# huggingface/gym-genesis

Measured on AMD Instinct MI355X. Metric: env-steps/sec (num_envs x sim-steps/sec), CubePick-v0 @ num_envs=4096, higher is better.
Workload: dtype f32

## Files before the change

gym-genesis_amd/csrc/mir_api.hip:

```cpp
#include <hip/hip_runtime.h>
#include <hip/hip_ext.h>

#include <cstdio>
#include <cstdlib>
#include <cstring>
#include <ctime>
#include <new>

#include "mir_host.h"
#include "mir_model.h"
#include "mir_scene.h"
#include "mir_spec_pick.h"
#include "mir_step.h"
#include "mir_step64.h"

using namespace mir_host;

static_assert((int)RK_FULL == (int)STEP_FULL && (int)RK_POST == (int)STEP_POST && (int)RK_ROTATED == (int)STEP_ROTATED && (int)RK_HEAVY48 == (int)STEP_HEAVY48 &&
              (int)RK_POST48 == (int)STEP_POST48 && (int)RK_ROTATED_LIST == (int)STEP_ROTATED_LIST, "mir_route.h numbers its launches like StepKind");

namespace {

thread_local char g_err[512] = "";

// ... 122 lines not shown
  snprintf(g_err, sizeof g_err, fmt, detail);
  return code;
}
int mir_host::hip_fail(hipError_t e, const char* what) {
  snprintf(g_err, sizeof g_err, "%s: %s", what, hipGetErrorString(e));
  return MIR_E_HIP;
}

int mir_host::launch(MirScene* h, const Outs& o, void* stream) {
  int rc;
  const bool sense = o.mode == 1 && (o.cf_ncon || o.cf_flags || o.cf_ids || o.cf_geom || o.cf_force || o.cf_link);
  if (!step_keeps_pre(o.kind) && o.mode != 2 && !sense) h->pre_valid = 0;
  const bool integrates = o.mode == 0 && step_integrates(o.kind);
  if (integrates && !step_completes_counted_step(o.kind)) h->state_version++;
  const bool wr_poses = o.poses || (h->poses_live && integrates);
  if (o.mode == 2 && o.poses) h->poses_current = 1;
  else if (integrates && o.kind != STEP_LIST48) h->poses_current = (h->kernel == 64 || wr_poses) && !o.ar.episode_len;
  if (h->kernel == 16) {
    StepArgs a;
    memset(&a, 0, sizeof a);
    a.model = h->dm;
    a.qpos = h->qpos; a.qvel = h->qvel; a.target = h->target; a.qacc_ws = h->qacc_ws;
    a.poses = wr_poses ? h->poses : nullptr;
    a.early_stats = h->early_stats; a.no_early_mask = h->no_early_mask;
    a.term_bad = h->pin_dev ? reinterpret_cast<uint32_t*>(h->pin_dev + h->pin_flag_off + 16) : nullptr;
    a.term_wstride = h->term_wstride;
    a.diag = (o.diag && h->diag_on) ? h->diag : nullptr;
    a.B = h->B; a.qst = h->hm.qstride; a.nu = h->hm.nu; a.features = (h->hm.has_convex ? FEAT_CONVEX : 0) | (h->hm.use_sap ? FEAT_CONVEX | FEAT_SAP : 0) | ((h->spec_pick && (!wr_poses || step_spec_stores_poses(o.kind))) ? FEAT_SPEC : 0);
    a.action = o.action; a.agent_pos = o.agent_pos; a.env_state = o.env_state; a.reward = o.reward; a.terminated = o.terminated;
    a.out_M = o.out_M; a.out_bias = o.out_bias; a.out_qas = o.out_qas; a.out_qacc = o.out_qacc; a.out_xpos = o.out_xpos; a.out_xquat = o.out_xquat;
    a.rows = o.rows; a.row_stride = o.row_stride; a.mode = o.mode; a.n_steps = o.n_steps; a.prof = o.prof;
    a.act_step = o.act_step; a.rows_step = o.rows_step; a.ar = o.ar;
    a.term_host = o.term_host; a.term_tag = o.term_tag; a.done_ticket = o.done_ticket; a.done_flag = o.done_flag; a.done_seq = o.done_seq;
    a.kind = o.kind; a.pre = h->pre;
    a.exact = o.exact; a.over_cap = o.over_cap;
    a.pre_big = step_uses_pre_big(o.kind) ? h->xc.res.pre_big : nullptr;
    a.next_host = o.next_host;
    a.cf_ncon = o.cf_ncon; a.cf_flags = o.cf_flags; a.cf_ids = o.cf_ids; a.cf_geom = o.cf_geom; a.cf_force = o.cf_force; a.cf_link = o.cf_link;
    if (step_forward_only(o.kind)) a.features &= ~FEAT_SPEC;
    if (o.env_list) { a.env_list = o.env_list; a.B = o.nlist; }
    if (o.kind == STEP_LIST48) a.term_wstride = 1;
    rc = mir_launch_step(&a, (hipStream_t)stream);
  } else {
    StepArgs64 a;
    memset(&a, 0, sizeof a);
    a.model = h->dm64;
    a.qpos = h->qpos; a.qvel = h->qvel; a.target = h->target; a.qacc_ws = h->qacc_ws;
// ... 54 lines not shown
namespace {

int create_device_state(MirScene* h, const GeomTab& gt, const float* row, size_t row_bytes) {
  DeviceGuard guard(h->device);
  const PlumbTab& t = h->pt;
  const size_t B = (size_t)h->B;
  const size_t qst = t.qst, vst = t.vst, pst = t.pst;
  HIPCHK(hipMalloc((void**)&h->dm, sizeof(DevModel)));
  HIPCHK(hipMalloc((void**)&h->dm64, sizeof(DevModel64)));
  HIPCHK(hipMalloc((void**)&h->dpt, sizeof(PlumbTab)));
  HIPCHK(hipMalloc((void**)&h->dgeom, sizeof(GeomTab)));
  HIPCHK(hipMalloc((void**)&h->qpos, B * qst * sizeof(float)));
  HIPCHK(hipMalloc((void**)&h->qvel, B * vst * sizeof(float)));
  HIPCHK(hipMalloc((void**)&h->target, B * vst * sizeof(float)));
  HIPCHK(hipMalloc((void**)&h->qacc_ws, B * vst * sizeof(float)));
  HIPCHK(hipMalloc((void**)&h->diag, B * 4 * sizeof(int32_t)));
  HIPCHK(hipMalloc((void**)&h->poses, B * 2 * pst * 4 * sizeof(float)));
  HIPCHK(hipMalloc((void**)&h->fkvalid, B * sizeof(int32_t)));
  HIPCHK(hipMalloc((void**)&h->done_ticket, 64));
  HIPCHK(hipMalloc((void**)&h->scratch_row, row_bytes));
  if (h->kernel == 16) HIPCHK(hipMalloc((void**)&h->pre, B * K16_PRE_STRIDE * sizeof(float)));
  h->spec_pick = h->kernel == 16 && SpecPick::matches(h->hm) && !getenv("MIR_NO_SPEC");
  h->no_early_mask = getenv("MIR_NO_EARLY_MASK") ? 1 : 0;
  HIPCHK(hipMalloc((void**)&h->early_stats, early_words(h) * sizeof(uint32_t)));
  HIPCHK(hipMemset(h->early_stats, 0, early_words(h) * sizeof(uint32_t)));
  if (h->kernel == 64) {
    h->cost_stride = (int)(((B + 63) / 64) * 64);
    HIPCHK(hipMalloc((void**)&h->cost, 2 * (size_t)h->cost_stride));
    HIPCHK(hipMemset(h->cost, 0, 2 * (size_t)h->cost_stride));
  }
  h->term_wstride = h->kernel == 16 ? 16 : 0;
  h->pin_flag_off = h->term_wstride ? ((B + 3) / 4) * 4 * (size_t)h->term_wstride : ((B + 63) / 64) * 64;
  h->pin_flag_off = (h->pin_flag_off + 63) / 64 * 64;
  const size_t pin_bytes = h->pin_flag_off + 64;
  HIPCHK(hipHostMalloc((void**)&h->pin_host, pin_bytes, hipHostMallocMapped | hipHostMallocCoherent));
  memset(h->pin_host, 0, pin_bytes);
  HIPCHK(hipHostGetDevicePointer((void**)&h->pin_dev, h->pin_host, 0));
  HIPCHK(hipMemcpy(h->dm, &h->hm, sizeof(DevModel), hipMemcpyHostToDevice));
  HIPCHK(hipMemcpy(h->dm64, &h->hm64, sizeof(DevModel64), hipMemcpyHostToDevice));
  HIPCHK(hipMemcpy(h->dpt, &h->pt, sizeof(PlumbTab), hipMemcpyHostToDevice));
  HIPCHK(hipMemcpy(h->dgeom, &gt, sizeof(GeomTab), hipMemcpyHostToDevice));
  for (int g = 0; g < gt.ngeom; g++) h->render_round |= gt.g_type[g] == MIR_GEOM_SPHERE || gt.g_type[g] == MIR_GEOM_CAPSULE;
  HIPCHK(hipMemcpy(h->scratch_row, row, row_bytes, hipMemcpyHostToDevice));
  hipLaunchKernelGGL(k_fill_rows, dim3(nblk((long)B * qst)), dim3(TPB), 0, 0, h->qpos, h->scratch_row, (int)qst, h->B);
  HIPCHK(hipGetLastError());
  HIPCHK(hipMemset(h->qvel, 0, B * vst * sizeof(float)));
// ... 829 lines not shown
```

gym-genesis_amd/csrc/mir_scene.h:

```cpp
#pragma once
#include <stdint.h>

#include "mir_model.h"
#include "mir_model64.h"
#include "mir_route.h"

struct ExactRes {
  int32_t *ovf_list_host, *ovf_list_dev;
  uint8_t *ovf_term_host, *ovf_term_dev;
  int32_t *perm_host[2], *perm_dev[2];
  void* ovf_stream;
  void* ovf_event;
  int ovf_event_live;
  void* ovf_waited_stream;
  void* main_event;
  void* light_event;
  float* pre_big;
  uint32_t *next_host, *next_dev;
  unsigned long long* xr_stats;
  int32_t* xr_count;
  int32_t *xr_list, *xr_list2, *xr_start;
  unsigned long long xr_calls;
};

// ... 6 lines not shown
  ExactStats stats;
};

struct MirScene {
  int device;
  int B;
  int kernel;
  DevModel hm;
  DevModel64 hm64;
  HostConsts hc;
  PlumbTab pt;
  int nbody, nv, nq, nu, ngeom, npair, agent_dim, env_dim;
  DevModel* dm;
  DevModel64* dm64;
  PlumbTab* dpt;
  GeomTab* dgeom;
  float *qpos, *qvel, *target, *qacc_ws, *poses;
  int32_t *diag, *fkvalid;
  uint8_t* cost = nullptr;
  int cost_par = 0;
  int cost_stride = 0;
  uint32_t* early_stats = nullptr;
  int no_early_mask = 0;
  int spec_pick = 0;
  float* prims;
  int* bins = nullptr;
  size_t bins_cap = 0;
  int render_th = 0;
  int render_generic = 0;
  int render_round = 0;
  unsigned long long* zbuf = nullptr;
  size_t zbuf_cap = 0;
  unsigned* vis = nullptr;
  size_t vis_cap = 0;
  unsigned long long state_version = 0;
  int poses_live = 0;
  int poses_current = 0;
  float* scratch_row;
  uint8_t* pin_host;
  size_t pin_flag_off = 0;
  int term_wstride = 0;
  uint8_t* pin_dev;
  uint32_t* done_ticket;
  uint32_t seq;
  uint32_t tag;
  int sync_mode;
// ... 22 lines not shown
```

gym-genesis_amd/csrc/mir_step.h:

```cpp
#pragma once
#include <hip/hip_runtime.h>
#include <stdint.h>

#include "mir_model.h"

enum : int { FEAT_PLAIN = 0 , FEAT_CONVEX = 1, FEAT_SAP = 2, FEAT_SPEC = 4 };

enum StepKind : int {
  STEP_SINGLE = 0,
  STEP_LOOP = 1,
  STEP_FULL = 2,
  STEP_PRE = 3,
  STEP_POST = 4,
  STEP_ROTATED = 5,
  STEP_LIST48 = 6,
  STEP_HEAVY48 = 7,
  STEP_POST48 = 9,
  STEP_PRE48 = 10,
  STEP_ROTATED_LIST = 11,
  STEP_XR16 = 12,
  STEP_XR48 = 13,
  STEP_SENSE48 = 14,
};

constexpr int step_cpl(int k) { return (k == STEP_LIST48 || k == STEP_HEAVY48 || k == STEP_POST48 || k == STEP_PRE48 || k == STEP_XR48 || k == STEP_SENSE48) ? 3 : 1; }
constexpr bool step_big(int k) { return step_cpl(k) > 1; }
constexpr bool step_fused_next_pre(int k) { return k == STEP_LIST48; }
constexpr bool step_packed(int k) { return step_big(k) || k == STEP_ROTATED_LIST; }
constexpr bool step_rotated(int k) { return k == STEP_ROTATED || k == STEP_POST48 || k == STEP_ROTATED_LIST; }
constexpr bool step_first_pass_only(int k) { return k == STEP_POST48 || k == STEP_ROTATED_LIST; }
constexpr bool step_pre_only(int k) { return k == STEP_PRE || k == STEP_PRE48; }
constexpr bool step_post_only(int k) { return k == STEP_POST; }
constexpr bool step_forward_only(int k) { return k == STEP_SENSE48; }
constexpr bool step_has_loop(int k) { return k == STEP_LOOP || k == STEP_FULL || k == STEP_XR16; }
constexpr bool step_rows_only(int k) { return k == STEP_LOOP || k == STEP_XR16; }
constexpr bool step_exact_rollout(int k) { return k == STEP_XR16 || k == STEP_XR48; }
constexpr int step_waves(int k) { return (step_has_loop(k) || step_post_only(k)) ? 1 : 2; }
constexpr int step_block(int k) { return 64 * step_waves(k); }
constexpr int step_wpe_min(int k) { return (step_rotated(k) && !step_big(k)) ? 2 : 1; }
constexpr int step_wpe_max(int k) { return (step_rotated(k) && !step_big(k)) ? 2 : (step_big(k) ? 1 : 10); }
constexpr bool step_defers(int k) { return k == STEP_SINGLE || k == STEP_POST || k == STEP_ROTATED || k == STEP_ROTATED_LIST || k == STEP_XR16 || step_big(k); }
constexpr bool step_reads_env_list(int k) { return k == STEP_PRE || k == STEP_ROTATED_LIST || step_big(k); }
constexpr bool step_sends_host_bytes(int k) { return k != STEP_LOOP && !step_forward_only(k); }
constexpr bool step_early_bytes_in_solver(int k) { return k == STEP_SINGLE || k == STEP_ROTATED || k == STEP_POST48 || k == STEP_ROTATED_LIST; }
constexpr bool step_spec_stores_poses(int k) { return step_rotated(k) || step_big(k); }
constexpr bool step_integrates(int k) { return !step_pre_only(k) && !step_forward_only(k); }
constexpr bool step_keeps_pre(int k) { return step_pre_only(k) || k == STEP_LIST48; }
constexpr bool step_completes_counted_step(int k) { return k == STEP_LIST48 || k == STEP_ROTATED_LIST; }
constexpr bool step_uses_pre_big(int k) { return k == STEP_LIST48 || k == STEP_POST48 || k == STEP_PRE48; }

struct StepArgs {
  const DevModel* model;
  float* qpos;
  float* qvel;
  float* target;
  float* qacc_ws;
  float* poses;
  const float* action;
  float* agent_pos;
  float* env_state;
  float* reward;
  uint8_t* terminated;
  uint8_t* term_host;
// ... 17 lines not shown
  int B;
  int qst, nu;
  int mode;
  int n_steps;
  int features;
  int kind;
  float* pre;
  uint32_t* early_stats;
  uint32_t* term_bad;
  int no_early_mask;
  int term_wstride;
  int exact;
  int over_cap;
  const int32_t* env_list;
  float* pre_big;
  uint32_t* next_host;
  int32_t* xr_list;
  int32_t* xr_count;
  int32_t* xr_list2;
  int32_t* xr_count2;
  int32_t* xr_start;
  unsigned long long* xr_stats;
  int xr_step;
  int32_t* cf_ncon;
  uint8_t* cf_flags;
  int32_t* cf_ids;
  float* cf_geom;
  float* cf_force;
  float* cf_link;
};
#ifndef XR_TIER2
#define XR_TIER2 (1 << 20)
#endif
#define K48_HEAD 0
#define K48_CMETA 4
#define K48_JB (K48_CMETA + 4 * MIR_MAX_CONTACT)
#define K48_STRIDE (((K48_JB + 48 * MIR_MAX_CONTACT) + 15) / 16 * 16)
#define K48_MAGIC 0x42494721
#define K16_PRE_MROW 0
#define K16_PRE_BIAS 256
#define K16_PRE_HEAD 272
#define K16_PRE_CMETA 276
#define K16_PRE_JB (K16_PRE_CMETA + 4 * K16_MAX_CONTACT)
#define K16_PRE_STRIDE (((K16_PRE_JB + 52 * K16_MAX_CONTACT) + 15) / 16 * 16)


// ... 3 lines not shown
```

gym-genesis_amd/csrc/mir_step.hip:

```cpp
#include <hip/hip_runtime.h>

#include <type_traits>
#include <stdint.h>

#include "mir_model.h"
#include "mir_step.h"
#include "mir_spec_pick.h"

#define G MIR_G
#include "mir_dev.h"
#include "mir_convex.h"
#define EPB 4
#define JST 52
#define MSTR 20
#define JB_SKEW 8
#define JBROW(Sx, c) (&(Sx).Jb_[(c) * JST + jbs])
static_assert(K16_MAX_CONTACT == G, "lane c owns contact c (one contact per lane; the step_big kinds keep CPL = 3 per lane)");

#ifdef MIR_PROFILE_SINGLE
#define STAMP(k) do { if (a.prof && !prof_mute && (int)blockIdx.x == prof_blk && threadIdx.x == 0) a.prof[k] = __builtin_readcyclecounter(); } while (0)
#define ITSTAMP(it, k) do { if ((it) < 8) STAMP(64 + 8 * (it) + (k)); } while (0)
#define HSTAMP(k) do { if (a.prof && !prof_mute && (int)blockIdx.x == prof_blk && threadIdx.x == 64) a.prof[k] = __builtin_readcyclecounter(); } while (0)
#else
#define HSTAMP(k) do { } while (0)
#define STAMP(k) do { if (a.prof && blockIdx.x == 0 && threadIdx.x == 0) a.prof[k] = __builtin_readcyclecounter(); } while (0)
#define ITSTAMP(it, k) do { } while (0)
#endif

#ifdef MIR_PROFILE_SINGLE
#define TERMSTAMP() do { if (a.prof && threadIdx.x == 0 && (blockIdx.x & 7) == (unsigned)(prof_blk & 7)) atomicMax(&a.prof[130], (unsigned long long)__builtin_amdgcn_s_memrealtime()); } while (0)
#else
#define TERMSTAMP() do { } while (0)
#endif
namespace {

struct DynScratch {
  float cddq[G][8];
  float cinert[G][12], crb[G][12];
  float cvel[G][8], cfrc[G][8];
};
template <int CPL>
struct ColScratchT {
  float gpos[K16_MAX_GEOM][4], gquat[K16_MAX_GEOM][4];
  int cand[G];
  int cmap[G * CPL];
  union {
    float stage[G][8][4];
// ... 35 lines not shown
    struct {
      DynScratch dyn;
      ColScratchT<CPL> col;
    };
    struct {
      ContactArraysT<CPL> con;
      float Jb_[MAXCON * JST + JB_SKEW];
    };
  };
};
typedef EnvLdsT<1> EnvLds;
static_assert(sizeof(EnvLds) == 2280 * 4, "the env block of the one-contact-per-lane instantiations (JB_SKEW above counts on 2280 dwords = 8 mod 32)");
static_assert(sizeof(ContactArraysT<1>) <= sizeof(DynScratch), "the contact arrays must not reach the collision staging area");
static_assert(sizeof(ContactArraysT<1>) + (G * JST + JB_SKEW) * sizeof(float) <= sizeof(DynScratch) + sizeof(ColScratchT<1>), "the skewed Jacobian rows must fit the union");
static_assert(EPB * sizeof(EnvLds) + sizeof(ModelTab) + K16_MAX_VERT * 16 <= 40960, "four workgroups per CU: 160 KB of LDS / 4 (hull vertices included)");
static_assert(EPB * sizeof(EnvLdsT<3>) + sizeof(ModelTab) + K16_MAX_VERT * 16 <= 81920, "the list instantiation (three contacts per lane): two workgroups per CU");

struct BodyK {
  int jtype, qadr;
  V3 pos, axis;
  Q4 quat;
};

template <bool SKIPFREE = false, class ENV>
__device__ __forceinline__ void group_fk(ENV& S, int lane, int nb, uint64_t parents, const BodyK& k, int row4) {
  V3 P = v3(0, 0, 0);
  Q4 Qx = Q4{1, 0, 0, 0};
  int anc = 0;
  const bool mine = lane < nb && !(SKIPFREE && k.jtype == MIR_JNT_FREE);
  if (lane > 0 && lane < nb && mine) {
    Qx = k.quat;
    P = k.pos;
    if (k.jtype == MIR_JNT_REVOLUTE) {
      float ang = S.qpos[k.qadr], sn, cs;
      sincos_pi2(0.5f * ang, &sn, &cs);
      Qx = qmul(k.quat, Q4{cs, k.axis.x * sn, k.axis.y * sn, k.axis.z * sn});
    } else if (k.jtype == MIR_JNT_PRISMATIC) {
      P = k.pos + qrot(k.quat, S.qpos[k.qadr] * k.axis);
    } else if (k.jtype == MIR_JNT_FREE) {
      P = ld3(&S.qpos[k.qadr]);
      Qx = qnormalize(ld4(&S.qpos[k.qadr + 3]));
    }
    anc = (int)((parents >> (4 * lane)) & 15u);
  }
#pragma unroll 1
  for (int round = 0; round < 4; round++) {
    if (!__any(anc > 0)) break;
    const int src = row4 + ((anc > 0 ? anc : lane) << 2);
    const V3 pa = v3(lane_gather(src, P.x), lane_gather(src, P.y), lane_gather(src, P.z));
    const Q4 qa = Q4{lane_gather(src, Qx.w), lane_gather(src, Qx.x), lane_gather(src, Qx.y), lane_gather(src, Qx.z)};
    const int nxt = lane_gather(src, anc);
    if (anc > 0) {
      P = pa + qrot(qa, P);
      Qx = qmul(qa, Qx);
      anc = nxt;
    }
  }
  if (mine) {
    st3v(S.xpos[lane], P);
    st4v(S.xquat[lane], Qx);
  }
// ... 166 lines not shown
```

gym-genesis_amd/csrc/mir_step_body.inc:

```
  constexpr bool ROT = step_rotated(VARIANT), FIRSTONLY = step_first_pass_only(VARIANT);
  constexpr bool BIGV = step_big(VARIANT), BIG2 = step_fused_next_pre(VARIANT);
  constexpr bool PRE = step_pre_only(VARIANT), POST = step_post_only(VARIANT);
  constexpr bool SINGLE = !step_has_loop(VARIANT), DUAL = step_waves(VARIANT) == 2;
  constexpr bool XR = step_exact_rollout(VARIANT);
  constexpr bool DEFER = step_defers(VARIANT);
  constexpr bool FWD = step_forward_only(VARIANT);
  constexpr int MAXCON = G * CPL;
  static_assert(CPL == step_cpl(VARIANT), "the kind fixes the contacts per lane");
  static_assert(JST == 52 && K16_PRE_STRIDE >= K16_PRE_JB + JST * K16_MAX_CONTACT, "pre-buffer layout");
  typedef EnvLdsT<CPL> EnvLds;
  constexpr bool CONVEX = (FEAT & FEAT_CONVEX) != 0, SAP = (FEAT & FEAT_SAP) != 0, SPEC = (FEAT & FEAT_SPEC) != 0;
  __shared__ __attribute__((aligned(16))) EnvLds s_env[EPB];
#define CFB(Sx, c) (CPL == 1 ? (Sx).con.cfb[CPL == 1 ? (c) : 0] : (Sx).con.cpos[c])
  __shared__ __attribute__((aligned(16))) ModelTab T;
  __shared__ __attribute__((aligned(16))) float s_hull[CONVEX ? K16_MAX_VERT : 1][4];
  __shared__ int s_help[CPL > 1 ? 4 : 1];
  const DevModel* __restrict__ m = a.model;
  const int tid = threadIdx.x & 63;
  const int wave = threadIdx.x >> 6;
#ifdef MIR_PROFILE_SINGLE
  const int prof_blk = a.prof ? (int)a.prof[63] : -1;
#else
  const int prof_blk = 0;
#endif
  [[maybe_unused]] bool prof_mute = false;
  STAMP(24);
  if (a.prof && (int)blockIdx.x == prof_blk && threadIdx.x == 0) a.prof[26] = __builtin_amdgcn_s_memrealtime();
  constexpr int TAB_NQ = (int)(sizeof(ModelTab) / 16), TAB_NPASS = (TAB_NQ + 63) / 64;
  f4 tabtmp[TAB_NPASS];
  if (wave == 0) {
    const f4* src = reinterpret_cast<const f4*>(&m->tab);
#pragma unroll
    for (int k = 0; k < TAB_NPASS; k++) tabtmp[k] = src[min(tid + 64 * k, TAB_NQ - 1)];
  }
  f4 hulltmp = {0, 0, 0, 0};
  if (CONVEX && wave == 0) hulltmp = reinterpret_cast<const f4*>(&m->hverts[0][0])[min(tid, K16_MAX_VERT - 1)];
  const int lane = tid & (G - 1);
  const int row4 = (tid & ~(G - 1)) << 2;
  const int grp = tid >> 4;
// ... 700 lines not shown
      stv(c + 8, f4{W[0][2] - mass * r.x * r.z, W[1][2] - mass * r.y * r.z, 0.0f, 0.0f});
    } else {
      stv(c, f4{0, 0, 0, 0}); stv(c + 4, f4{0, 0, 0, 0}); stv(c + 8, f4{0, 0, 0, 0});
    }
  };
  if (DUAL && wave == 1) {
    auto helper_cinert = [&](int pass_no) {
      const f4 h0 = *reinterpret_cast<const f4*>(m->lanek_t[0][lane]), h4 = *reinterpret_cast<const f4*>(m->lanek_t[4][lane]);
      const f4 h5 = *reinterpret_cast<const f4*>(m->lanek_t[5][lane]), h6 = *reinterpret_cast<const f4*>(m->lanek_t[6][lane]);
      const float hib[6] = {h5.x, h5.y, h5.z, h5.w, h6.x, h6.y};
      cinert_store(lane < nb && lane > 0, hib, v3(h4.x, h4.y, h4.z), h4.w, __float_as_int(h0.z));
      WSYNC();
      if (lane == 0) __hip_atomic_store(&S.cin_ready, pass_no, __ATOMIC_RELEASE, __HIP_MEMORY_SCOPE_WORKGROUP);
    };
    auto fk_consts = [&](BodyK& hk) {
      const f4 h0 = *reinterpret_cast<const f4*>(m->lanek_t[0][lane]), h1 = *reinterpret_cast<const f4*>(m->lanek_t[1][lane]);
      const f4 h2 = *reinterpret_cast<const f4*>(m->lanek_t[2][lane]), h3 = *reinterpret_cast<const f4*>(m->lanek_t[3][lane]);
      hk.jtype = __float_as_int(h0.x); hk.qadr = __float_as_int(h0.y);
      hk.pos = v3(h1.x, h1.y, h1.z);
      hk.quat = Q4{h2.x, h2.y, h2.z, h2.w};
      hk.axis = v3(h3.x, h3.y, h3.z);
    };
    const uint64_t hparents = m->parents;
    bool ovf_h = false;
    if (ROT) {
      {
        const float* pre = a.pre + (size_t)env * K16_PRE_STRIDE;
        const f4 head = *reinterpret_cast<const f4*>(pre + K16_PRE_HEAD);
        int nc = __float_as_int(head.x);
        int cplw = __float_as_int(head.y);
        const int pts_h = (cplw >> 20) & 255;
        bool big_h = false;
        if constexpr (CPL > 1) {
          big_h = pts_h > K16_MAX_CONTACT && pts_h <= MAXCON && __float_as_int(head.z) == K48_MAGIC && a.pre_big != nullptr;
          if (!big_h && nc != pts_h) { cplw |= 255 << 20; nc = 0; }
        }
        ovf_h = ((cplw >> 20) & 255) > defer_above;
        if constexpr (CPL > 1) {
          const float* big = a.pre_big + (size_t)env * K48_STRIDE;
          f4 h2 = {0, 0, 0, 0};
          if (big_h) { h2 = *reinterpret_cast<const f4*>(big + K48_HEAD); nc = __float_as_int(h2.x); }
          if (lane == 0) { S.ncon = nc; S.coupled = cplw; S.ncand = 0; S.conB[0] = (cplw >> 1) & 0xffff; S.conB[1] = __float_as_int(h2.y); S.conB[2] = __float_as_int(h2.z); }
          if (big_h) {
#pragma unroll
            for (int sl = 0; sl < CPL; sl++)
              if (lane + G * sl < nc) stv(S.con.cmeta[lane + G * sl], *reinterpret_cast<const f4*>(big + K48_CMETA + 4 * (lane + G * sl)));
            bigrows_load(big, nc, S);
          } else {
            if (lane < nc) stv(S.con.cmeta[lane], *reinterpret_cast<const f4*>(pre + K16_PRE_CMETA + 4 * lane));
            jrows_load(pre, nc, (uint64_t)__float_as_uint(head.z) | ((uint64_t)__float_as_uint(head.w) << 32), S);
          }
        } else {
          if (lane == 0) { S.ncon = nc; S.coupled = cplw; S.ncand = 0; }
          if (lane < nc) stv(S.con.cmeta[lane], *reinterpret_cast<const f4*>(pre + K16_PRE_CMETA + 4 * lane));
          jrows_load(pre, nc, (uint64_t)__float_as_uint(head.z) | ((uint64_t)__float_as_uint(head.w) << 32), S);
        }
        WSYNC();
        HSTAMP(54);
        __syncthreads();
        float hp[G];
        hess_full(hp, nc);
#pragma unroll
        for (int q = 0; q < 4; q++) stv(&S.M[lane][4 * q], f4{hp[4 * q], hp[4 * q + 1], hp[4 * q + 2], hp[4 * q + 3]});
        HSTAMP(55);
        __syncthreads();
        helper_newton();
      }
      BodyK hk;
      fk_consts(hk);
      __syncthreads();
      HSTAMP(56);
      group_fk<true>(S, lane, nb, hparents, hk, row4);
      HSTAMP(57);
      __syncthreads();
      if (FIRSTONLY) return;
    } else {
      const float hq_lo = lane < a.qst ? a.qpos[(size_t)env * a.qst + lane] : 0.0f;
      const float hq_hi = lane + G < a.qst ? a.qpos[(size_t)env * a.qst + lane + G] : 0.0f;
      BodyK hk;
      fk_consts(hk);
      if (lane < a.qst) S.qpos[lane] = hq_lo;
      if (lane + G < a.qst) S.qpos[lane + G] = hq_hi;
      WSYNC();
      group_fk(S, lane, nb, hparents, hk, row4);
    }
    HSTAMP(40);
    if (!ROT) __syncthreads();
    HSTAMP(41);
    auto pre_store = [&]() {
      if (valid && !ovf_h) {
        float* pre = a.pre + (size_t)env * K16_PRE_STRIDE;
        const int nc = S.ncon;
        if (CPL == 1 || nc <= K16_MAX_CONTACT) {
          const uint64_t qm = jrows_store(pre, nc, S);
          if (lane == 0) *reinterpret_cast<f4*>(pre + K16_PRE_HEAD) = f4{__int_as_float(nc), __int_as_float(S.coupled), __uint_as_float((uint32_t)qm), __uint_as_float((uint32_t)(qm >> 32))};
          if (lane < nc) *reinterpret_cast<f4*>(pre + K16_PRE_CMETA + 4 * lane) = ldv(S.con.cmeta[lane]);
// ... 4 lines not shown
              float* big = a.pre_big + (size_t)env * K48_STRIDE;
              bigrows_store(big, nc, S);
#pragma unroll
              for (int sl = 0; sl < CPL; sl++)
                if (lane + G * sl < nc) *reinterpret_cast<f4*>(big + K48_CMETA + 4 * (lane + G * sl)) = ldv(S.con.cmeta[lane + G * sl]);
              if (lane == 0) *reinterpret_cast<f4*>(big + K48_HEAD) = f4{__int_as_float(nc), __int_as_float(S.conB[1]), __int_as_float(S.conB[2]), 0.0f};
            }
          }
          if (lane == 0) *reinterpret_cast<f4*>(pre + K16_PRE_HEAD) = f4{__int_as_float(0), __int_as_float(S.coupled), __int_as_float(bigok ? K48_MAGIC : 0), 0.0f};
        }
      }
#ifdef MIR_PROFILE_SINGLE
      if (a.prof && threadIdx.x == 64 && (blockIdx.x & 7) == (unsigned)(prof_blk & 7)) atomicMax(&a.prof[31], (unsigned long long)__builtin_amdgcn_s_memrealtime());
#endif
    };
    helper_cinert(1);
    const int cnt = collide_detect(1);
    HSTAMP(42);
    const int pts0 = contacts_build(cnt, PRE || ROT || BIGV);
    if (BIGV && !ROT && !PRE) ovf_h = pts0 > defer_above;
    HSTAMP(45);
    __syncthreads();
    HSTAMP(46);
    {
      if (PRE || ROT) {
        if (VARIANT == STEP_PRE48 && a.next_host) {
          const unsigned long long fb = __ballot(valid && pts0 > a.over_cap && lane == 0);
          if (tid == 0) {
            const uint32_t bits = (uint32_t)(fb & 1u) | (uint32_t)(fb >> 16 & 1u) << 8 | (uint32_t)(fb >> 32 & 1u) << 16 | (uint32_t)(fb >> 48 & 1u) << 24;
            __hip_atomic_store(a.next_host + blockIdx.x, bits | (a.term_tag << 1) * 0x01010101u, __ATOMIC_RELAXED, __HIP_MEMORY_SCOPE_SYSTEM);
          }
        }
        pre_store();
        return;
      }
      float hp[G];
      hess_full(hp, S.ncon);
#pragma unroll
      for (int q = 0; q < 4; q++) stv(&S.M[lane][4 * q], f4{hp[4 * q], hp[4 * q + 1], hp[4 * q + 2], hp[4 * q + 3]});
    }
    HSTAMP(47);
    __syncthreads();
    helper_newton();
    if (FWD) return;
    if (fksplit) {
      BodyK hk;
      fk_consts(hk);
      __syncthreads();
      group_fk<true>(S, lane, nb, hparents, hk, row4);
      __syncthreads();
    }
    if constexpr (BIG2) {
      HSTAMP(142);
      prof_mute = true;
      helper_cinert(2);
      const int cnt2 = collide_detect(2);
      contacts_build(cnt2, true);
      __syncthreads();
      pre_store();
#ifdef MIR_PROFILE_SINGLE
      if (a.prof && (int)blockIdx.x == prof_blk && threadIdx.x == 64) a.prof[141] = __builtin_readcyclecounter();
#endif
    }
    return;
  }

  const bool isbody = lane < nb && lane > 0;
  const bool isdof = lane < nv;
  const uint64_t parents = m->parents;
  f4 lk[12];
  {
#pragma unroll
// ... 30 lines not shown
    f4* dst = reinterpret_cast<f4*>(&T);
#pragma unroll
    for (int k = 0; k < TAB_NPASS; k++)
      if (tid + 64 * k < TAB_NQ) dst[tid + 64 * k] = tabtmp[k];
    if (CONVEX && tid < K16_MAX_VERT) stv(s_hull[tid], hulltmp);
  }
  if (!DUAL || ROT) {
    if (lane < a.qst) S.qpos[lane] = q_lo;
    if (lane + G < a.qst) S.qpos[lane + G] = q_hi;
  }
  S.qvel[lane] = qv_in;
  S.qacc_ws[lane] = ws_in;
  if (a.action) {
    const float mine = __shfl(au, (tid & ~(G - 1)) + (d_uadr >= 0 ? d_uadr : 0));
    if (isdof && d_uadr >= 0) tg = mine;
  }
  S.target[lane] = tg;
  if (lane == 0) {
    if (!ROT) { S.ncon = 0; S.ncand = 0; }
    S.cin_ready = 0;
    if constexpr (CPL > 1) { S.bp_ready = 0; S.bb_done = 0; }
  }
  if constexpr (CPL > 1) { if (tid == 0) { s_help[0] = 0; s_help[1] = 0; s_help[2] = 0; } }
  WSYNC();

  STAMP(0);
  if (!DUAL && !POST) group_fk(S, lane, nb, parents, bk, row4);
  STAMP(1);
  STAMP(48);
  if (DUAL && !ROT) __syncthreads();
  const int nsteps = (ROT || BIG2) ? 2 : (SINGLE ? 1 : (a.mode == 0 ? a.n_steps : (a.mode == 1 ? 1 : 0)));
  if (PRE || (SPEC && !step_spec_stores_poses(VARIANT))) a.poses = nullptr;
  if (SINGLE) { a.mode = 0; a.act_step = 0; if (VARIANT != STEP_XR48) { a.rows_step = 0; a.ar.episode_len = nullptr; } a.out_M = a.out_bias = a.out_qas = a.out_qacc = a.out_xpos = a.out_xquat = nullptr;
#ifndef MIR_PROFILE_SINGLE
    a.prof = nullptr;
#endif
  }
  if (VARIANT == STEP_XR48) { a.poses = nullptr; a.agent_pos = a.env_state = a.reward = nullptr; a.terminated = a.term_host = nullptr; a.done_ticket = nullptr; }
  if (step_rows_only(VARIANT)) { a.mode = 0; a.out_M = a.out_bias = a.out_qas = a.out_qacc = a.out_xpos = a.out_xquat = nullptr; a.prof = nullptr; a.agent_pos = a.env_state = a.reward = nullptr; a.terminated = a.term_host = nullptr; a.done_ticket = nullptr; }
  const int eb = mdl_eef, ob = mdl_obj;
  const int ad = 7 + mdl_ngrip;
  auto column = [&](int c) -> float {
    const V3 pe = ld3v(S.xpos[eb]), po = ld3v(S.xpos[ob]);
    const V3 df = pe - po;
    if (c < 3) return S.xpos[eb][c];
    if (c < 7) return S.xquat[eb][c - 3];
// ... 329 lines not shown
    float lsg = 0.0f, lD = 0.0f, laref = 0.0f;
    if (d_limited) {
      float q = S.qpos[d_qadr];
      const f4 l0 = ldv(&T.d_lim[lane][0]);
      float dlo = q - l0.x, dhi = l0.y - q;
      float pos = 0.0f;
      if (dlo < 0.0f) { pos = dlo; lsg = 1.0f; }
      else if (dhi < 0.0f) { pos = dhi; lsg = -1.0f; }
      if (lsg != 0.0f) {
        const f4 l1 = ldv(&T.d_lim[lane][4]), l2 = ldv(&T.d_lim[lane][8]);
        float imp = impedance(l1.y, l1.z, l1.w, l2.x, l2.y, pos);
        float Rr = fmaxf((1.0f - imp) / imp * l0.z, 1e-15f);
        lD = 1.0f / Rr;
        laref = -l1.x * (lsg * S.qvel[lane]) - l0.w * imp * pos;
      }
    }
    WSYNC();
    if (BIGV && !post_now) {
      __syncthreads();
      jac_build(2, 4);
    }
    STAMP(50);
    if (DUAL && (!post_now || ROT)) __syncthreads();
    STAMP(52);
    const int ncon = S.ncon;
    bool iscon[CPL];
    float cmu[CPL], cD[CPL];
    float aref[CPL][4], jar[CPL][4];
#pragma unroll
    for (int sl = 0; sl < CPL; sl++) {
      iscon[sl] = lane + G * sl < ncon;
      cmu[sl] = 0.0f; cD[sl] = 0.0f;
#pragma unroll
      for (int r = 0; r < 4; r++) { aref[sl][r] = 0.0f; jar[sl][r] = 0.0f; }
    }
    const JRow jrow = jrow_load(JBROW(S, iscon[0] ? lane : 0));
    auto jd3 = [&](int sl, float x, float& dn, float& d1, float& d2) __attribute__((always_inline)) {
      if (sl == 0) jdot3_bc(jrow, x, dn, d1, d2);
      else jdot3_bc(jrow_load(JBROW(S, iscon[sl] ? lane + G * sl : 0)), x, dn, d1, d2);
    };
#pragma unroll
    for (int sl = 0; sl < CPL; sl++) {
      if (sl > 0 && !__any(iscon[sl])) continue;
      float vn, v1, v2;
      jd3(sl, S.qvel[lane], vn, v1, v2);
      if (iscon[sl]) {
// ... 18 lines not shown
        for (int i = lane; i < qst; i += G) a.qpos[(size_t)env * qst + i] = S.qpos[i];
        a.qvel[(size_t)env * G + lane] = S.qvel[lane];
        a.qacc_ws[(size_t)env * G + lane] = S.qacc_ws[lane];
        if (lane == 0) {
          if (a.ar.episode_len) { a.ar.episode_len[env] = eplen; a.ar.cursor[env] = epcur; }
          a.xr_start[env] = step;
          a.xr_list[atomicAdd(a.xr_count, 1)] = env;
        }
      }
      ovf_env = ovf_env || now;
    }
    if (BIGV) over_env = a.over_cap > 0 && ((cpl >> 20) & 255) > a.over_cap;
    const int hsplit = __any((cpl & 1) != 0) ? 0 : mdl_split;
    const bool sep = mdl_split > 0 && (cpl & 1) == 0;
    const bool dofB = sep && lane >= mdl_split;
    bool conB[CPL];
    conB[0] = sep && ((cpl >> (1 + lane)) & 1) != 0;
    if constexpr (CPL > 1) {
#pragma unroll
      for (int sl = 1; sl < CPL; sl++) conB[sl] = sep && ((S.conB[sl] >> lane) & 1) != 0;
    }
    bool done = nefc == 0;
    float qacc = qas, Ma = 0.0f, ljar = 0.0f;
    {
      const float ws = S.qacc_ws[lane];
      const float dq = isdof ? ws - qas : 0.0f;
      float d_ws = 0.5f * rowdot_bc(mrow, dq) * dq, d_sm = 0.0f;
      const float ljs = lsg * qas - laref, ljw = lsg * ws - laref;
      if (lsg != 0.0f) {
        if (ljs < 0.0f) d_sm += 0.5f * lD * ljs * ljs;
        if (ljw < 0.0f) d_ws += 0.5f * lD * ljw * ljw;
      }
      float js[CPL][4], jw[CPL][4], k_df[CPL];
#pragma unroll
      for (int sl = 0; sl < CPL; sl++) {
        float k_ws = 0.0f, k_sm = 0.0f;
#pragma unroll
        for (int r = 0; r < 4; r++) { js[sl][r] = 0.0f; jw[sl][r] = 0.0f; }
        if (sl == 0 || __any(iscon[sl])) {
          float sn, s1, s2, wn, w1, w2;
          jd3(sl, qas, sn, s1, s2);
          jd3(sl, ws, wn, w1, w2);
          if (iscon[sl]) {
            const float mu = cmu[sl];
            js[sl][0] = sn + mu * s1 - aref[sl][0]; js[sl][1] = sn - mu * s1 - aref[sl][1]; js[sl][2] = sn + mu * s2 - aref[sl][2]; js[sl][3] = sn - mu * s2 - aref[sl][3];
            jw[sl][0] = wn + mu * w1 - aref[sl][0]; jw[sl][1] = wn - mu * w1 - aref[sl][1]; jw[sl][2] = wn + mu * w2 - aref[sl][2]; jw[sl][3] = wn - mu * w2 - aref[sl][3];
// ... 3 lines not shown
              if (jw[sl][r] < 0.0f) k_ws += 0.5f * cD[sl] * jw[sl][r] * jw[sl][r];
            }
          }
        }
        k_df[sl] = k_ws - k_sm;
      }
      const float d_df = d_ws - d_sm;
      float dfA = (dofB ? 0.0f : d_df) + (conB[0] ? 0.0f : k_df[0]), dfB = (dofB ? d_df : 0.0f) + (conB[0] ? k_df[0] : 0.0f);
#pragma unroll
      for (int sl = 1; sl < CPL; sl++) { dfA += conB[sl] ? 0.0f : k_df[sl]; dfB += conB[sl] ? k_df[sl] : 0.0f; }
      bool usewsA = gsum_u(dfA) < 0.0f, usewsB = usewsA;
      if (__any(sep)) usewsB = gsum_u(dfB) < 0.0f;
      const bool usewsd = dofB ? usewsB : usewsA;
      qacc = usewsd ? ws : qas;
      ljar = usewsd ? ljw : ljs;
#pragma unroll
      for (int sl = 0; sl < CPL; sl++) {
        const bool usewsc = conB[sl] ? usewsB : usewsA;
#pragma unroll
        for (int r = 0; r < 4; r++) jar[sl][r] = usewsc ? jw[sl][r] : js[sl][r];
      }
      const float Mab = rowdot_bc(mrow, qacc);
      Ma = isdof ? Mab : 0.0f;
    }
    STAMP(7);
    int niter = 0;
    const float tol = mdl_tolerance, scale = mdl_scale;
    constexpr float gfl = 16.0f * 5.96e-8f;
    float gfw;
    {
      const float f2 = Ma * Ma + qfs * qfs;
      const float FA2 = gsum(dofB ? 0.0f : f2);
      float FB2 = FA2;
      if (__any(sep)) FB2 = gsum(dofB ? f2 : 0.0f);
      gfw = 1.0f / fmaxf(dofB ? FB2 : FA2, 1e-30f);
    }
    float hkeep[G];
#pragma unroll
    for (int j = 0; j < G; j++) hkeep[j] = isdof ? mrow[j] : (j == lane ? 1.0f : 0.0f);
    float oldlact = 0.0f;
    bool term_sent = false;
    uint32_t term_bits = 0u;
    float d_gw = 0.0f;
    if (term_bound) d_gw = m->lanek_t[11][lane][3];
    unsigned prevbits[CPL];
#pragma unroll
// ... 251 lines not shown
#pragma unroll
        for (int sl = 1; sl < CPL; sl++) pB += conB[sl] ? pimc[sl] : 0.0f;
        const float gainB = gsum_u(pB + (dofB ? piml : 0.0f)) - (0.5f * alpha * alpha * AB + alpha * BB);
        const float gainA = improvement - gainB;
        const bool okA = gainA > 0.0f, okB = gainB > 0.0f;
        if (need && !(okA && okB)) {
          ald = (dofB ? okB : okA) ? alpha : 0.0f;
#pragma unroll
          for (int sl = 0; sl < CPL; sl++) alc[sl] = (conB[sl] ? okB : okA) ? alpha : 0.0f;
          improvement = (okA ? gainA : 0.0f) + (okB ? gainB : 0.0f);
          partial = okA != okB;
        }
      }
      if (!need && !(improvement > 0.0f)) {
        ald = 0.0f;
#pragma unroll
        for (int sl = 0; sl < CPL; sl++) alc[sl] = 0.0f;
        improvement = 0.0f;
      }
      const float moved = gsum((isdof && qacc + ald * sv != qacc) ? 1.0f : 0.0f);
      const bool stagnant = it > 0 && gw > 0.5f * gprev && gw < 4.0f * gfl;
      gprev = gw;
      if (!done && !partial && (moved == 0.0f || stagnant)) { done = true; niter = it + 1; }
      if (!done) {
        qacc += ald * sv;
        Ma += ald * mv;
        ljar += ald * ljv;
#pragma unroll
        for (int sl = 0; sl < CPL; sl++)
#pragma unroll
        for (int r = 0; r < 4; r++) jar[sl][r] += alc[sl] * jv[sl][r];
        niter = it + 1;
        if (!partial && scale * improvement < tol) done = true;
      }
      {
        const float gnew = fabsf(1.0f - alpha) * gn, gwnew = fabsf(1.0f - alpha) * gw;
        if (!done && ncross == 0.0f && (scale * gnew < tol || gwnew < gfl)) done = true;
      }
#ifdef MIR_DEBUG_TRACE
      if (a.prof && valid && env == (int)a.prof[255] && it < 8) {
        float* tr = reinterpret_cast<float*>(a.prof + 256) + (it * G + lane) * 16;
        tr[0] = qacc; tr[1] = jar[0][0]; tr[2] = jar[0][1]; tr[3] = jar[0][2]; tr[4] = jar[0][3]; tr[5] = (float)prevbits[0]; tr[6] = g; tr[7] = sv;
        tr[8] = alpha; tr[9] = ald; tr[10] = alc[0]; tr[11] = improvement; tr[12] = ncross; tr[13] = done ? 1.0f : 0.0f; tr[14] = (float)flipmask[0]; tr[15] = partial ? 1.0f : 0.0f;
      }
#endif
      WSYNC();
      if (it == 0) STAMP(21);
      ITSTAMP(it, 7);
    }
    if (DUAL && (!post_now || ROT) && !met4) __syncthreads();
    if constexpr (CPL > 1) { if (tid == 0) __hip_atomic_store(&s_help[0], -1, __ATOMIC_RELEASE, __HIP_MEMORY_SCOPE_WORKGROUP); }
    if constexpr (FWD) {
      WSYNC();
#pragma unroll
      for (int sl = 0; sl < CPL; sl++) {
        const int k = lane + G * sl;
        V3 F = v3(0, 0, 0);
        uint32_t ids = 0u;
        if (iscon[sl]) {
          float f[4];
#pragma unroll
          for (int r = 0; r < 4; r++) f[r] = jar[sl][r] < 0.0f ? -cD[sl] * jar[sl][r] : 0.0f;
          const V3 cn = ld3v(&S.con.cfrm[k][0]), c1 = ld3v(&S.con.cfrm[k][4]), c2 = ld3v(&S.con.cfrm[k][8]);
          F = (f[0] + f[1] + f[2] + f[3]) * cn + (cmu[sl] * (f[0] - f[1])) * c1 + (cmu[sl] * (f[2] - f[3])) * c2;
          ids = S.con.cmask[k][3];
        }
        if (valid && a.cf_force) st3(&a.cf_force[((size_t)env * MAXCON + k) * 3], F);
        stv(&S.con.cref[k][0], f4{F.x, F.y, F.z, __uint_as_float(ids)});
      }
      WSYNC();
      if (a.cf_link) {
        V3 acc = v3(0, 0, 0);
// ... 3 lines not shown
          const float sg = ((int)(ids >> 24) == lane ? 1.0f : 0.0f) - ((int)(ids >> 16 & 255u) == lane ? 1.0f : 0.0f);
          acc = acc + sg * v3(v.x, v.y, v.z);
        }
        if (valid && lane < nb) st3(&a.cf_link[((size_t)env * nb + lane) * 3], acc);
      }
      if (valid && lane == 0) {
        if (a.cf_ncon) a.cf_ncon[env] = ncon;
        if (a.cf_flags) a.cf_flags[env] = ovf_env ? 1 : 0;
      }
      return 2;
    }
    if (a.out_qacc && valid && isdof && step == 0) a.out_qacc[(size_t)env * nv + lane] = qacc;
    if (a.diag && valid && !ovf_env && lane == 0) {
      a.diag[(size_t)env * 4 + 0] = ncon;
      a.diag[(size_t)env * 4 + 1] = nefc;
      a.diag[(size_t)env * 4 + 2] = niter;
      a.diag[(size_t)env * 4 + 3] = S.ncand | (cpl >> 20 & 255) << 8;
    }
    STAMP(8);
    if (a.mode != 0) return 1;

    WSYNC();
    if (isdof) {
      S.qvel[lane] += dt * qacc;
      S.qacc_ws[lane] = qacc;
    }
    WSYNC();
    if (isdof) {
      const float qd = S.qvel[lane];
      if (d_kind < 2) S.qpos[d_qadr] += dt * qd;
      else if (d_kind == 2) S.qpos[T.b_info[d_body][2] + d_axis_k] += dt * qd;
    }
    if (step_sends_host_bytes(VARIANT) && a.term_host && term_early) {
      WSYNC();
      const bool tn = valid && !ovf_env && above(S.qpos[mdl_obj_qadr + 2], mdl_reward_z);
      const unsigned long long tb = __ballot(tn && lane == 0), db = __ballot(ovf_env && valid && lane == 0), ob = BIGV ? __ballot(over_env && valid && lane == 0) : 0ull;
      if (tid == 0) {
        const uint32_t bits = (uint32_t)(tb & 1u) | (uint32_t)(tb >> 16 & 1u) << 8 | (uint32_t)(tb >> 32 & 1u) << 16 | (uint32_t)(tb >> 48 & 1u) << 24 |
                              (uint32_t)(db & 1u) << 7 | (uint32_t)(db >> 16 & 1u) << 15 | (uint32_t)(db >> 32 & 1u) << 23 | (uint32_t)(db >> 48 & 1u) << 31 |
                              (uint32_t)(ob & 1u) << 6 | (uint32_t)(ob >> 16 & 1u) << 14 | (uint32_t)(ob >> 32 & 1u) << 22 | (uint32_t)(ob >> 48 & 1u) << 30;
        if (!term_sent || bits != term_bits)
          __hip_atomic_store(reinterpret_cast<uint32_t*>(a.term_host) + (size_t)blockIdx.x * a.term_wstride, bits | (a.term_tag << 1) * 0x01010101u, __ATOMIC_RELAXED,
                             __HIP_MEMORY_SCOPE_SYSTEM);
        if (term_sent && bits != term_bits) {
          if (a.early_stats) atomicAdd(a.early_stats + 1, 1u);
          if (a.term_bad) __hip_atomic_store(a.term_bad, 1u, __ATOMIC_RELAXED, __HIP_MEMORY_SCOPE_SYSTEM);
        }
      }
      if (!term_sent) { STAMP(30); TERMSTAMP(); }
    }
    if (fksplit) {
      WSYNC();
      __syncthreads();
    }
    if (isdof) {
      if (d_kind == 3 && d_axis_k == 0) {
        const int da = T.b_info[d_body][3], qa = T.b_info[d_body][2];
        V3 w = v3(S.qvel[da + 3], S.qvel[da + 4], S.qvel[da + 5]);
        float wn = sqrtf(dot(w, w));
        float ang = wn * dt;
        if (ang > 1e-15f) {
          float sn, cs;
          sincos_pi2(0.5f * ang, &sn, &cs);
          V3 ax = (1.0f / wn) * w;
          Q4 dq = {cs, ax.x * sn, ax.y * sn, ax.z * sn};
          st4(&S.qpos[qa + 3], qnormalize(qmul(dq, ld4(&S.qpos[qa + 3]))));
        }
      }
    }
    WSYNC();
    STAMP(9);
    if (a.diag) {
      const bool nf = (lane < qst && nonfinite(S.qpos[lane])) || (lane + G < qst && nonfinite(S.qpos[lane + G])) || nonfinite(S.qvel[lane]);
      const bool bad = ((uint32_t)(__ballot(nf) >> (grp * G)) & 0xffffu) != 0u;
      bad_acc = bad_acc || bad;
      if (valid && !ovf_env && lane == 0) {
        a.diag[(size_t)env * 4 + 3] = S.ncand | (cpl >> 20 & 255) << 8 | (bad_acc ? 1 << 30 : 0);
        if (bad && a.early_stats) atomicAdd(a.early_stats, 1u);
      }
    }
    if (fksplit) {
      if (isbody && bk.jtype == MIR_JNT_FREE) {
        st3v(S.xpos[lane], ld3(&S.qpos[bk.qadr]));
        st4v(S.xquat[lane], qnormalize(ld4(&S.qpos[bk.qadr + 3])));
      }
      WSYNC();
      __syncthreads();
    } else {
      group_fk(S, lane, nb, parents, bk, row4);
    }
    if (a.rows && a.rows_step && (step + 1 < nsteps || a.ar.episode_len) && valid && (!XR || !ovf_env)) {
      float* row = a.rows + (size_t)step * a.rows_step + (size_t)env * a.row_stride;
      for (int c = lane; c < ad + 13; c += G) row[c] = column(c);
    }
    if (a.ar.episode_len) {
      const bool term = above(S.xpos[ob][2], mdl_reward_z);
      const int len = eplen + 1;
      const bool trunc = !term && a.ar.max_len > 0 && len >= a.ar.max_len;
      const bool done = term || trunc;
      if (valid && (!XR || !ovf_env) && lane == 0 && a.rows && a.row_stride > ad + 13)
        a.rows[(size_t)step * a.rows_step + (size_t)env * a.row_stride + ad + 13] = trunc ? 1.0f : 0.0f;
      eplen = done ? 0 : len;
      WSYNC();
      if (done) {
        S.qvel[lane] = 0.0f;
        S.qacc_ws[lane] = 0.0f;
        if (isdof) {
          const int ai = m->d_armidx[lane];
          if (ai >= 0) {
            const float v = a.ar.arm_qpos[(size_t)env * m->n_arm_q + ai];
            S.qpos[d_qadr] = v;
// ... 34 lines not shown
```

Baseline: 191.5 million.

## Speculate helper-wave forward kinematics on intermediate solver accelerations

In the two-wave single and rotated step variants, the helper wave no longer waits for the Newton solve to finish before running forward kinematics. The main wave publishes each updated qacc through a shared-memory sequence counter. The helper recomputes joint positions by Euler integration and reruns FK each time a new value appears, until a final flag is set. The main wave runs at raised priority during the solve, and one workgroup barrier after integration is dropped when speculation is on. This aims to hide FK latency behind solver iterations, at the cost of extra spin-polling, redundant FK work, and added shared-memory writes on every iteration.

```diff
diff --git a/gym-genesis_amd/csrc/mir_api.hip b/gym-genesis_amd/csrc/mir_api.hip
--- a/gym-genesis_amd/csrc/mir_api.hip
+++ b/gym-genesis_amd/csrc/mir_api.hip
@@ -168,7 +168,7 @@
     a.model = h->dm;
     a.qpos = h->qpos; a.qvel = h->qvel; a.target = h->target; a.qacc_ws = h->qacc_ws;
     a.poses = wr_poses ? h->poses : nullptr;
-    a.early_stats = h->early_stats; a.no_early_mask = h->no_early_mask;
+    a.early_stats = h->early_stats; a.no_early_mask = h->no_early_mask; a.no_spec_pose = h->no_spec_pose;
     a.term_bad = h->pin_dev ? reinterpret_cast<uint32_t*>(h->pin_dev + h->pin_flag_off + 16) : nullptr;
     a.term_wstride = h->term_wstride;
     a.diag = (o.diag && h->diag_on) ? h->diag : nullptr;
@@ -269,6 +269,7 @@
   if (h->kernel == 16) HIPCHK(hipMalloc((void**)&h->pre, B * K16_PRE_STRIDE * sizeof(float)));
   h->spec_pick = h->kernel == 16 && SpecPick::matches(h->hm) && !getenv("MIR_NO_SPEC");
   h->no_early_mask = getenv("MIR_NO_EARLY_MASK") ? 1 : 0;
+  h->no_spec_pose = getenv("MIR_NO_SPEC_POSE") ? 1 : 0;
   HIPCHK(hipMalloc((void**)&h->early_stats, early_words(h) * sizeof(uint32_t)));
   HIPCHK(hipMemset(h->early_stats, 0, early_words(h) * sizeof(uint32_t)));
   if (h->kernel == 64) {
diff --git a/gym-genesis_amd/csrc/mir_scene.h b/gym-genesis_amd/csrc/mir_scene.h
--- a/gym-genesis_amd/csrc/mir_scene.h
+++ b/gym-genesis_amd/csrc/mir_scene.h
@@ -52,6 +52,7 @@
   int cost_stride = 0;
   uint32_t* early_stats = nullptr;
   int no_early_mask = 0;
+  int no_spec_pose = 0;
   int spec_pick = 0;
   float* prims;
   int* bins = nullptr;
diff --git a/gym-genesis_amd/csrc/mir_step.h b/gym-genesis_amd/csrc/mir_step.h
--- a/gym-genesis_amd/csrc/mir_step.h
+++ b/gym-genesis_amd/csrc/mir_step.h
@@ -39,6 +39,9 @@
 constexpr int step_block(int k) { return 64 * step_waves(k); }
 constexpr int step_wpe_min(int k) { return (step_rotated(k) && !step_big(k)) ? 2 : 1; }
 constexpr int step_wpe_max(int k) { return (step_rotated(k) && !step_big(k)) ? 2 : (step_big(k) ? 1 : 10); }
+constexpr bool step_speculates_pose(int k) { return k == STEP_SINGLE || k == STEP_ROTATED; }
+static_assert(step_waves(STEP_SINGLE) == 2 && step_cpl(STEP_SINGLE) == 1 && !step_has_loop(STEP_SINGLE) && !step_forward_only(STEP_SINGLE), "step_speculates_pose");
+static_assert(step_waves(STEP_ROTATED) == 2 && step_cpl(STEP_ROTATED) == 1 && !step_has_loop(STEP_ROTATED) && !step_forward_only(STEP_ROTATED), "step_speculates_pose");
 constexpr bool step_defers(int k) { return k == STEP_SINGLE || k == STEP_POST || k == STEP_ROTATED || k == STEP_ROTATED_LIST || k == STEP_XR16 || step_big(k); }
 constexpr bool step_reads_env_list(int k) { return k == STEP_PRE || k == STEP_ROTATED_LIST || step_big(k); }
 constexpr bool step_sends_host_bytes(int k) { return k != STEP_LOOP && !step_forward_only(k); }
@@ -102,6 +105,7 @@
   int32_t* xr_start;
   unsigned long long* xr_stats;
   int xr_step;
+  int no_spec_pose;
   int32_t* cf_ncon;
   uint8_t* cf_flags;
   int32_t* cf_ids;
diff --git a/gym-genesis_amd/csrc/mir_step.hip b/gym-genesis_amd/csrc/mir_step.hip
--- a/gym-genesis_amd/csrc/mir_step.hip
+++ b/gym-genesis_amd/csrc/mir_step.hip
@@ -21,8 +21,10 @@
 #define STAMP(k) do { if (a.prof && !prof_mute && (int)blockIdx.x == prof_blk && threadIdx.x == 0) a.prof[k] = __builtin_readcyclecounter(); } while (0)
 #define ITSTAMP(it, k) do { if ((it) < 8) STAMP(64 + 8 * (it) + (k)); } while (0)
 #define HSTAMP(k) do { if (a.prof && !prof_mute && (int)blockIdx.x == prof_blk && threadIdx.x == 64) a.prof[k] = __builtin_readcyclecounter(); } while (0)
+#define PSTAMP(k) STAMP(k)
 #else
 #define HSTAMP(k) do { } while (0)
+#define PSTAMP(k) do { } while (0)
 #define STAMP(k) do { if (a.prof && blockIdx.x == 0 && threadIdx.x == 0) a.prof[k] = __builtin_readcyclecounter(); } while (0)
 #define ITSTAMP(it, k) do { } while (0)
 #endif
@@ -104,8 +106,10 @@
   Q4 quat;
 };
 
-template <bool SKIPFREE = false, class ENV>
-__device__ __forceinline__ void group_fk(ENV& S, int lane, int nb, uint64_t parents, const BodyK& k, int row4) {
+#define EULER_AXIS(x, h, v) ((x) += (h) * (v))
+
+template <bool SKIPFREE = false, bool QGIVEN = false, class ENV>
+__device__ __forceinline__ void group_fk(ENV& S, int lane, int nb, uint64_t parents, const BodyK& k, int row4, float qj = 0.0f) {
   V3 P = v3(0, 0, 0);
   Q4 Qx = Q4{1, 0, 0, 0};
   int anc = 0;
@@ -114,11 +118,11 @@
     Qx = k.quat;
     P = k.pos;
     if (k.jtype == MIR_JNT_REVOLUTE) {
-      float ang = S.qpos[k.qadr], sn, cs;
+      float ang = QGIVEN ? qj : S.qpos[k.qadr], sn, cs;
       sincos_pi2(0.5f * ang, &sn, &cs);
       Qx = qmul(k.quat, Q4{cs, k.axis.x * sn, k.axis.y * sn, k.axis.z * sn});
     } else if (k.jtype == MIR_JNT_PRISMATIC) {
-      P = k.pos + qrot(k.quat, S.qpos[k.qadr] * k.axis);
+      P = k.pos + qrot(k.quat, (QGIVEN ? qj : S.qpos[k.qadr]) * k.axis);
     } else if (k.jtype == MIR_JNT_FREE) {
       P = ld3(&S.qpos[k.qadr]);
       Qx = qnormalize(ld4(&S.qpos[k.qadr + 3]));
diff --git a/gym-genesis_amd/csrc/mir_step_body.inc b/gym-genesis_amd/csrc/mir_step_body.inc
--- a/gym-genesis_amd/csrc/mir_step_body.inc
+++ b/gym-genesis_amd/csrc/mir_step_body.inc
@@ -15,6 +15,8 @@
   __shared__ __attribute__((aligned(16))) ModelTab T;
   __shared__ __attribute__((aligned(16))) float s_hull[CONVEX ? K16_MAX_VERT : 1][4];
   __shared__ int s_help[CPL > 1 ? 4 : 1];
+  constexpr bool SPECP = step_speculates_pose(VARIANT);
+  __shared__ int s_spec[SPECP ? 2 : 1];
   const DevModel* __restrict__ m = a.model;
   const int tid = threadIdx.x & 63;
   const int wave = threadIdx.x >> 6;
@@ -761,8 +763,40 @@
       hk.axis = v3(h3.x, h3.y, h3.z);
     };
     const uint64_t hparents = m->parents;
+    [[maybe_unused]] const bool spec_on = SPECP && fksplit && !a.no_spec_pose;
+    [[maybe_unused]] float sp_q = 0.0f, sp_v = 0.0f;
+    [[maybe_unused]] int sp_dof = 0;
+    [[maybe_unused]] auto spec_snapshot = [&](const BodyK& k) {
+      const bool jointed = lane > 0 && lane < nb && (k.jtype == MIR_JNT_REVOLUTE || k.jtype == MIR_JNT_PRISMATIC);
+      sp_dof = jointed ? T.b_info[lane][3] : 0;
+      sp_q = jointed ? S.qpos[k.qadr] : 0.0f;
+      sp_v = S.qvel[sp_dof];
+    };
+    [[maybe_unused]] auto spec_fk_loop = [&](const BodyK& k) {
+      if constexpr (SPECP) {
+        int have = 0;
+        for (;;) {
+          const int fin = __builtin_amdgcn_readfirstlane(__hip_atomic_load(&s_spec[1], __ATOMIC_ACQUIRE, __HIP_MEMORY_SCOPE_WORKGROUP));
+          const int seq = __builtin_amdgcn_readfirstlane(__hip_atomic_load(&s_spec[0], __ATOMIC_ACQUIRE, __HIP_MEMORY_SCOPE_WORKGROUP));
+          if (seq != have) {
+            float qd = sp_v, qj = sp_q;
+            EULER_AXIS(qd, dt, S.qacc_ws[sp_dof]);
+            EULER_AXIS(qj, dt, qd);
+            group_fk<true, true>(S, lane, nb, hparents, k, row4, qj);
+            have = seq;
+            HSTAMP(62);
+          } else if (fin != 0) {
+            break;
+          } else {
+            __builtin_amdgcn_s_sleep(1);
+          }
+        }
+        HSTAMP(39);
+      }
+    };
     bool ovf_h = false;
     if (ROT) {
+      BodyK hk;
       {
         const float* pre = a.pre + (size_t)env * K16_PRE_STRIDE;
         const f4 head = *reinterpret_cast<const f4*>(pre + K16_PRE_HEAD);
@@ -797,20 +831,27 @@
         WSYNC();
         HSTAMP(54);
         __syncthreads();
+        if (spec_on) fk_consts(hk);
         float hp[G];
         hess_full(hp, nc);
 #pragma unroll
         for (int q = 0; q < 4; q++) stv(&S.M[lane][4 * q], f4{hp[4 * q], hp[4 * q + 1], hp[4 * q + 2], hp[4 * q + 3]});
+        if (spec_on) spec_snapshot(hk);
         HSTAMP(55);
         __syncthreads();
         helper_newton();
       }
-      BodyK hk;
-      fk_consts(hk);
-      __syncthreads();
-      HSTAMP(56);
-      group_fk<true>(S, lane, nb, hparents, hk, row4);
-      HSTAMP(57);
+      if (spec_on) {
+        spec_fk_loop(hk);
+        HSTAMP(56);
+        HSTAMP(57);
+      } else {
+        fk_consts(hk);
+        __syncthreads();
+        HSTAMP(56);
+        group_fk<true>(S, lane, nb, hparents, hk, row4);
+        HSTAMP(57);
+      }
       __syncthreads();
       if (FIRSTONLY) return;
     } else {
@@ -861,6 +902,7 @@
     HSTAMP(45);
     __syncthreads();
     HSTAMP(46);
+    BodyK hk2;
     {
       if (PRE || ROT) {
         if (VARIANT == STEP_PRE48 && a.next_host) {
@@ -873,20 +915,28 @@
         pre_store();
         return;
       }
+      if (spec_on) fk_consts(hk2);
       float hp[G];
       hess_full(hp, S.ncon);
 #pragma unroll
       for (int q = 0; q < 4; q++) stv(&S.M[lane][4 * q], f4{hp[4 * q], hp[4 * q + 1], hp[4 * q + 2], hp[4 * q + 3]});
+      if (spec_on) spec_snapshot(hk2);
     }
     HSTAMP(47);
     __syncthreads();
     helper_newton();
     if (FWD) return;
-    if (fksplit) {
-      BodyK hk;
-      fk_consts(hk);
+    if (spec_on) {
+      spec_fk_loop(hk2);
+      HSTAMP(56);
+      HSTAMP(57);
       __syncthreads();
-      group_fk<true>(S, lane, nb, hparents, hk, row4);
+    } else if (fksplit) {
+      fk_consts(hk2);
+      __syncthreads();
+      HSTAMP(56);
+      group_fk<true>(S, lane, nb, hparents, hk2, row4);
+      HSTAMP(57);
       __syncthreads();
     }
     if constexpr (BIG2) {
@@ -963,6 +1013,7 @@
     if constexpr (CPL > 1) { S.bp_ready = 0; S.bb_done = 0; }
   }
   if constexpr (CPL > 1) { if (tid == 0) { s_help[0] = 0; s_help[1] = 0; s_help[2] = 0; } }
+  if constexpr (SPECP) { if (tid == 0) { s_spec[0] = 0; s_spec[1] = 0; } }
   WSYNC();
 
   STAMP(0);
@@ -1338,6 +1389,7 @@
     }
     STAMP(50);
     if (DUAL && (!post_now || ROT)) __syncthreads();
+    if constexpr (SPECP) __builtin_amdgcn_s_setprio(3);
     STAMP(52);
     const int ncon = S.ncon;
     bool iscon[CPL];
@@ -1402,6 +1454,15 @@
     }
     bool done = nefc == 0;
     float qacc = qas, Ma = 0.0f, ljar = 0.0f;
+    [[maybe_unused]] int spec_seq = 0;
+    [[maybe_unused]] auto spec_publish = [&]() {
+      if constexpr (SPECP) {
+        if (isdof) S.qacc_ws[lane] = qacc;
+        WSYNC();
+        spec_seq += 1;
+        if (tid == 0) __hip_atomic_store(&s_spec[0], spec_seq, __ATOMIC_RELAXED, __HIP_MEMORY_SCOPE_WORKGROUP);
+      }
+    };
     {
       const float ws = S.qacc_ws[lane];
       const float dq = isdof ? ws - qas : 0.0f;
@@ -1451,6 +1512,7 @@
       }
       const float Mab = rowdot_bc(mrow, qacc);
       Ma = isdof ? Mab : 0.0f;
+      spec_publish();
     }
     STAMP(7);
     int niter = 0;
@@ -1748,6 +1810,7 @@
       const bool stagnant = it > 0 && gw > 0.5f * gprev && gw < 4.0f * gfl;
       gprev = gw;
       if (!done && !partial && (moved == 0.0f || stagnant)) { done = true; niter = it + 1; }
+      [[maybe_unused]] const float qacc_was = qacc;
       if (!done) {
         qacc += ald * sv;
         Ma += ald * mv;
@@ -1763,6 +1826,7 @@
         const float gnew = fabsf(1.0f - alpha) * gn, gwnew = fabsf(1.0f - alpha) * gw;
         if (!done && ncross == 0.0f && (scale * gnew < tol || gwnew < gfl)) done = true;
       }
+      if constexpr (SPECP) { if (__any(isdof && qacc != qacc_was)) spec_publish(); }
 #ifdef MIR_DEBUG_TRACE
       if (a.prof && valid && env == (int)a.prof[255] && it < 8) {
         float* tr = reinterpret_cast<float*>(a.prof + 256) + (it * G + lane) * 16;
@@ -1774,6 +1838,8 @@
       if (it == 0) STAMP(21);
       ITSTAMP(it, 7);
     }
+    if constexpr (SPECP) { if (tid == 0) __hip_atomic_store(&s_spec[1], spec_seq + 1, __ATOMIC_RELAXED, __HIP_MEMORY_SCOPE_WORKGROUP); }
+    PSTAMP(38);
     if (DUAL && (!post_now || ROT) && !met4) __syncthreads();
     if constexpr (CPL > 1) { if (tid == 0) __hip_atomic_store(&s_help[0], -1, __ATOMIC_RELEASE, __HIP_MEMORY_SCOPE_WORKGROUP); }
     if constexpr (FWD) {
@@ -1823,13 +1889,13 @@
 
     WSYNC();
     if (isdof) {
-      S.qvel[lane] += dt * qacc;
+      EULER_AXIS(S.qvel[lane], dt, qacc);
       S.qacc_ws[lane] = qacc;
     }
     WSYNC();
     if (isdof) {
       const float qd = S.qvel[lane];
-      if (d_kind < 2) S.qpos[d_qadr] += dt * qd;
+      if (d_kind < 2) EULER_AXIS(S.qpos[d_qadr], dt, qd);
       else if (d_kind == 2) S.qpos[T.b_info[d_body][2] + d_axis_k] += dt * qd;
     }
     if (step_sends_host_bytes(VARIANT) && a.term_host && term_early) {
@@ -1852,7 +1918,7 @@
     }
     if (fksplit) {
       WSYNC();
-      __syncthreads();
+      if (!(SPECP && !a.no_spec_pose)) __syncthreads();
     }
     if (isdof) {
       if (d_kind == 3 && d_axis_k == 0) {
@@ -1886,8 +1952,12 @@
         st4v(S.xquat[lane], qnormalize(ld4(&S.qpos[bk.qadr + 3])));
       }
       WSYNC();
+      PSTAMP(36);
+      if constexpr (SPECP) __builtin_amdgcn_s_setprio(0);
       __syncthreads();
+      PSTAMP(37);
     } else {
+      if constexpr (SPECP) __builtin_amdgcn_s_setprio(0);
       group_fk(S, lane, nb, parents, bk, row4);
     }
     if (a.rows && a.rows_step && (step + 1 < nsteps || a.ar.episode_len) && valid && (!XR || !ovf_env)) {
```

Result: slower. 188.8 million (-1.4%).
